# NVlabs/EmerNeRF

Hardware: AMD Instinct MI355X
Metric: train rays/sec (8192-ray batch, 128 samples) (higher is better)
Workload: dtype f32

## Files before the change

### emernerf_amd/_lib.py

```python
from __future__ import annotations

import ctypes
import os
from ctypes import c_float, c_int, c_int32, c_int64, c_uint32, c_uint64, c_void_p

_PKG = os.path.dirname(os.path.abspath(__file__))
LIB_PATH = os.path.join(_PKG, "lib", "libemernerf_hip.so")
EMER_MAX_LEVELS = 32

F32, F16 = 0, 1
ACT_NONE, ACT_RELU, ACT_SIGMOID, ACT_TRUNC_EXP = 0, 1, 2, 3
STOT_TYPES = {"uniform": 0, "uniform_lindisp": 1, "lindisp": 2, "sqrt": 3, "log": 4, "uniform_lindisp_0": 5}


class GridDesc(ctypes.Structure):
    _fields_ = [
        ("n_dims", c_uint32), ("n_levels", c_uint32), ("n_features", c_uint32),
        ("log2_hashmap_size", c_uint32), ("base_resolution", c_uint32), ("per_level_scale", c_float),
        ("scale", c_float * EMER_MAX_LEVELS), ("res", c_uint32 * EMER_MAX_LEVELS),
        ("size", c_uint32 * EMER_MAX_LEVELS), ("offset", c_uint32 * EMER_MAX_LEVELS),
        ("hashed", c_uint32 * EMER_MAX_LEVELS), ("n_entries", c_uint32),
    ]


class EmerError(RuntimeError):
    pass


_P = c_void_p
_GP = ctypes.POINTER(GridDesc)

SIGNATURES = {
    "emer_profile_next": [_P, _P],
    "emer_grid_desc_init": [_GP, c_uint32, c_uint32, c_uint32, c_uint32, c_uint32, c_float],
    "emer_hashgrid_fwd": [_GP, _P, _P, c_int, _P, c_int64, c_int64, _P, c_int64, _P],
    "emer_hashgrid_bwd_params": [_GP, _P, _P, c_int64, c_int64, _P, c_int, c_int64, _P],
    "emer_hashgrid_bwd_params_sliced": [_GP, _P, _P, c_int64, c_int64, _P, _P, c_int64, _P],
    "emer_hashgrid_bwd_params_sliced_add": [_GP, _P, _P, c_int64, c_int64, _P, _P, c_int64, _P],
    "emer_hashgrid_bwd_params_sliced_levels": [_GP, _P, _P, c_int64, c_int64, _P, _P, c_int64, c_int32, c_int32, _P],
    "emer_hashgrid_sliced_split_level": [_GP],
    "emer_hashgrid_sliced_plan": [_GP, _P, _P],
    "emer_hashgrid_slice_masks": [_GP, _P, _P, c_int64, _P],
    "emer_hashgrid_sliced_supported": [_GP],
    "emer_hashgrid_mask_rows": [_P],
    "emer_hashgrid_bwd_input": [_GP, _P, _P, c_int, _P, c_int64, c_int64, _P, c_int64, _P],
    "emer_hashgrid_fwd_jac": [_GP, _P, _P, _P, c_int64, c_int64, _P, _P, c_int64, c_int64, _P],
    "emer_hashgrid_bwd_input_jac": [_GP, _P, _P, c_int64, c_int64, _P, c_int64, _P],
    "emer_layout_transpose": [_P, _P, c_int32, c_int64, c_int32, c_int, _P],
    "emer_contract_fwd": [_P, _P, c_int, _P, c_int64, _P],
    "emer_contract_bwd": [_P, _P, c_int, _P, _P, c_int64, _P],
    "emer_flow_warp_fwd": [_P, _P, _P, _P, _P, c_float, _P, c_int, _P, _P, c_int64, _P],
    "emer_flow_warp_bwd": [_P, _P, _P, _P, c_int, _P, _P, _P, c_int64, _P],
    "emer_ray_points": [_P, _P, _P, _P, _P, _P, c_int, _P, c_int, _P, c_int64, c_int32, _P],
    "emer_importance_sample": [_P, _P, c_int64, c_int32, c_int32, _P, _P, _P, _P, c_float, c_float, c_int, _P],
    "emer_importance_sample_points": [_P, _P, c_int64, c_int32, c_int32, _P, _P, _P, _P, c_float, c_float, c_int, _P, _P, _P, c_int, _P, _P, _P],
    "emer_stot": [_P, c_int64, c_float, c_float, c_int, _P, _P],
    "emer_prop_loss": [_P, _P, c_int32, _P, _P, c_int32, c_float, c_int, c_int64, c_float, _P, _P, c_int, _P, _P],
    "emer_reduce_sum": [_P, c_int64, c_int, _P, _P],
    "emer_scale": [_P, _P, c_float, _P, c_int64, _P],
    "emer_cast_f32_f16": [_P, _P, c_int64, _P],
    "emer_render_weights_fwd": [_P, _P, _P, c_int64, c_int32, _P, _P, _P, _P, _P, _P, _P, _P],
    "emer_render_weights_bwd": [_P, _P, _P, _P, _P, _P, _P, c_int64, c_int32, _P, _P],
    "emer_composite_rgb_fwd": [_P, _P, _P, _P, _P, c_int64, c_int32, _P, _P, _P, _P, _P, _P, _P, _P, _P, _P],
    "emer_composite_rgb_bwd": [_P, _P, _P, _P, _P, _P, _P, _P, _P, _P, _P, _P, c_int64, c_int32, _P, _P, _P, _P],
    "emer_blend_accumulate_fwd": [_P, _P, _P, _P, _P, _P, _P, c_int64, c_int32, _P, _P, _P],
    "emer_blend_accumulate_bwd": [_P, _P, _P, _P, _P, _P, _P, _P, _P, c_int64, c_int32, _P, _P, _P, _P, _P, _P, _P, _P],
    "emer_blend_accumulate_wide_fwd": [_P, _P, _P, _P, _P, _P, c_int64, c_int32, c_int32, _P, _P],
    "emer_blend_accumulate_wide_bwd": [_P, _P, _P, _P, _P, _P, _P, c_int64, c_int32, c_int32, _P, _P, _P, _P, _P, _P, _P],
    "emer_ray_epilogue_fwd": [_P, _P, _P, c_int64, _P, _P, _P, _P, _P],
    "emer_ray_epilogue_bwd": [_P, _P, _P, _P, _P, c_int64, _P, _P, _P],
    "emer_pixel_loss_fwd": [_P, _P, _P, _P, c_int64, c_float, c_float, _P, _P, _P],
    "emer_pixel_loss_bwd": [_P, _P, _P, _P, c_int64, c_float, c_float, _P, _P, _P, _P],
# ... 84 lines not shown
            try:
                fn = getattr(lib, name)
            except AttributeError:
                if ALLOW_MISSING_SYMBOLS:
                    continue
                raise
            fn.argtypes = argtypes
            fn.restype = restype
    lib.emer_last_error.restype = ctypes.c_char_p
    lib.emer_version.restype = c_int
    _lib = lib
    return lib


class KernelTimer:

    def __init__(self, names):
        self.names = set(names)
        self.events = {n: [] for n in self.names}
        self.tags = {n: [] for n in self.names}
        self.ns = {n: [] for n in self.names}
        self.tag = None

    def elapsed_us(self):
        import torch
        torch.cuda.synchronize()
        return {n: [a.elapsed_time(b) * 1e3 for a, b in ev] for n, ev in self.events.items()}


TIMER = None


_N_ARG = {"emer_hashgrid_fwd": 8, "emer_hashgrid_fwd_jac": 9, "emer_hashgrid_bwd_params_sliced": 7, "emer_hashgrid_bwd_params_sliced_add": 7,
          "emer_hashgrid_bwd_params_sliced_levels": 7, "emer_hashgrid_bwd_params": 7, "emer_hashgrid_bwd_input": 8, "emer_hashgrid_bwd_input_jac": 6}
_TIGHT = ("emer_hashgrid_fwd", "emer_hashgrid_fwd_jac", "emer_hashgrid_bwd_params_sliced", "emer_hashgrid_bwd_params_sliced_add", "emer_hashgrid_bwd_params_sliced_levels")


def call(name: str, *args) -> None:
    lib = load()
    t = TIMER
    if t is not None and name in t.names:
        import torch
        a, b = torch.cuda.Event(enable_timing=True), torch.cuda.Event(enable_timing=True)
        a.record()
        if name in _TIGHT:
            b.record()
            lib.emer_profile_next(c_void_p(a.cuda_event), c_void_p(b.cuda_event))
            rc = getattr(lib, name)(*args)
        else:
            rc = getattr(lib, name)(*args)
            b.record()
        t.events[name].append((a, b))
        tag = None
        if name.startswith("emer_hashgrid"):
            d = args[0]._obj
            tag = (d.n_dims, d.n_levels, d.n_features)
        t.tags[name].append(tag)
        t.ns[name].append(int(args[_N_ARG[name]]) if name in _N_ARG else None)
    else:
        rc = getattr(lib, name)(*args)
    if rc != 0:
        raise EmerError(f"{name} failed (rc={rc}): {lib.emer_last_error().decode()}")


def make_grid_desc(n_dims, n_levels, n_features, log2_hashmap_size, base_resolution, per_level_scale) -> GridDesc:
    d = GridDesc()
    call("emer_grid_desc_init", ctypes.byref(d), n_dims, n_levels, n_features, log2_hashmap_size,
         base_resolution, per_level_scale)
# ... 2 lines not shown
```

### emernerf_amd/csrc/hashgrid.hip

```cpp
#include "common.h"

namespace emer {

template <int F, typename PT>
__device__ __forceinline__ void load_feats(const PT *__restrict__ p, float (&v)[F]);

template <> __device__ __forceinline__ void load_feats<1, float>(const float *__restrict__ p, float (&v)[1]) { v[0] = p[0]; }
template <> __device__ __forceinline__ void load_feats<2, float>(const float *__restrict__ p, float (&v)[2]) {
    float2 t = *reinterpret_cast<const float2 *>(p); v[0] = t.x; v[1] = t.y;
}
template <> __device__ __forceinline__ void load_feats<4, float>(const float *__restrict__ p, float (&v)[4]) {
    float4 t = *reinterpret_cast<const float4 *>(p); v[0] = t.x; v[1] = t.y; v[2] = t.z; v[3] = t.w;
}
template <> __device__ __forceinline__ void load_feats<8, float>(const float *__restrict__ p, float (&v)[8]) {
    float4 a = reinterpret_cast<const float4 *>(p)[0], b = reinterpret_cast<const float4 *>(p)[1];
    v[0] = a.x; v[1] = a.y; v[2] = a.z; v[3] = a.w; v[4] = b.x; v[5] = b.y; v[6] = b.z; v[7] = b.w;
}
template <> __device__ __forceinline__ void load_feats<1, __half>(const __half *__restrict__ p, float (&v)[1]) { v[0] = __half2float(p[0]); }
template <> __device__ __forceinline__ void load_feats<2, __half>(const __half *__restrict__ p, float (&v)[2]) {
    float2 t = __half22float2(*reinterpret_cast<const __half2 *>(p)); v[0] = t.x; v[1] = t.y;
}
template <> __device__ __forceinline__ void load_feats<4, __half>(const __half *__restrict__ p, float (&v)[4]) {
    uint2 raw = *reinterpret_cast<const uint2 *>(p);
    float2 a = __half22float2(*reinterpret_cast<__half2 *>(&raw.x)), b = __half22float2(*reinterpret_cast<__half2 *>(&raw.y));
// ... 709 lines not shown
    (void)slice_want; (void)slice_bits;
    const bool on = (uint32_t)lane < count;
    const uint32_t e = on ? Qw[(q_head + (uint32_t)lane) % kPairQueue] : 0u;
    uint32_t n = e >> 8;
    uint32_t match = e & 0xFFu;
    asm volatile("" : "+v"(n));
    float xv[D], go[F], w[D];
    uint32_t gi[D], hd[D][2];
    load_x<D>(x, (int64_t)n, xv);
#pragma unroll
    for (int f = 0; f < F; ++f) go[f] = dl[(int64_t)n * sn + f];
    cell_of<D>(li, xv, gi, w);
    hash_terms<D>(gi, hd);
    add_pair<D, F>(acc, gi, w, hd, go, match, local_mask);
    while (__ballot(match != 0u)) add_pair<D, F>(acc, gi, w, hd, go, match, local_mask);
}

#ifndef EMER_PIPE_K
#define EMER_PIPE_K 2
#endif
template <int D, int F> constexpr int kPipeK() {
    constexpr int per = D + F + 1, k = 28 / per;
    return k > EMER_PIPE_K ? EMER_PIPE_K : (k < 1 ? 1 : k);
}
template <int D, int F, int K>
struct HitGroup {
    float xs[K][D], go[K][F];
    uint32_t ns[K];
    bool vld[K];
    uint32_t take;
};
constexpr int kScanWords = 64 + 64 + 32 + 32;

template <int D, int F>
__global__ __launch_bounds__(kSliceThreads) void hashgrid_bwd_params_sliced_kernel(const emer_grid_desc g, const SlicePlan plan,
                                                                                   const float *__restrict__ x,
                                                                                   const float *__restrict__ dout, int64_t sn, int64_t sl,
                                                                                   const uint64_t *__restrict__ masks,
                                                                                   uint32_t *__restrict__ work_ctr,
                                                                                   float *__restrict__ grad, int64_t N,
                                                                                   uint32_t accumulate) {
    extern __shared__ __attribute__((aligned(16))) double smem[];
    __shared__ uint32_t s_item;
    const uint32_t my_xcd = blockIdx.x & 7u;
    uint8_t *sel_lut = nullptr;
    if constexpr (use_select_lut<D>()) {
    sel_lut = reinterpret_cast<uint8_t *>(reinterpret_cast<uint64_t *>(smem + (size_t)plan.max_local * F) + (size_t)kSliceWaves * kScanWords)
                       + (size_t)kSliceWaves * kPairQueue * sizeof(uint32_t);
    for (uint32_t e = threadIdx.x; e < 2048u; e += kSliceThreads) {
        uint32_t b = e >> 3, k = e & 7u, pos = 0;
        for (uint32_t i = 0; i < 8u; ++i)
            if ((b >> i) & 1u) { if (k == 0u) { pos = i; break; } --k; }
        sel_lut[e] = (uint8_t)pos;
    }
    __syncthreads();
    }
  for (;;) {
    if (threadIdx.x == 0) {
        uint32_t it = 0xFFFFFFFFu;
        for (uint32_t t = 0; t < 8u; ++t) {
            const uint32_t xx = (my_xcd + t) & 7u;
            if (plan.items_per_xcd[xx] == 0u) continue;
            const uint32_t jj = atomicAdd(work_ctr + xx, 1u);
            if (jj < plan.items_per_xcd[xx]) { it = (xx << 24) | jj; break; }
        }
        s_item = it;
    }
    __syncthreads();
    const uint32_t item = s_item;
    __syncthreads();
    if (item == 0xFFFFFFFFu) return;
    const uint32_t xcd = item >> 24;
    uint32_t j = item & 0xFFFFFFu;
    j = ((((j >> plan.sched_shift) << 3) + xcd) << plan.sched_shift) + (j & ((1u << plan.sched_shift) - 1u));
    uint32_t level = 0, slice = 0, range = 0;
    for (uint32_t oi = 0; oi < g.n_levels; ++oi) {
        level = plan.order[oi];
        const uint32_t nb = plan.n_slices[level] * plan.n_ranges[level];
        if (j < nb) { slice = j % plan.n_slices[level]; range = j / plan.n_slices[level]; break; }
        j -= nb;
    }
    const LevelInfo li = level_info(g, level);
#ifdef EMER_SLICED_TRACE
    const unsigned long long trace_t0 = wall_clock64();
    unsigned long long trace_hits = 0;
#endif
    const bool dense_rt = !li.hashed;
    const bool pairable_rt = li.hashed && (li.size & (li.size - 1u)) == 0u && true;
    const bool run_reduced = pairable_rt && F >= 2 && li.res <= (uint32_t)EMER_RUN_RES;
    const bool consecutive = dense_rt || run_reduced || li.res > kStridedHitsMaxRes;
    const uint32_t shift = plan.shift[level], n_ranges = plan.n_ranges[level];
    const uint32_t first = slice << shift;
    const uint32_t n_local = ((li.size - first) < (1u << shift)) ? (li.size - first) : (1u << shift);
    const int64_t n_words = (N + 63) >> 6;
    const int64_t words_per_range = ceil_div_dev(n_words, (int64_t)n_ranges);
    const int64_t w_begin = (int64_t)range * words_per_range;
    const int64_t w_end = (w_begin + words_per_range < n_words) ? w_begin + words_per_range : n_words;

    double *acc = smem;
    const int wave = threadIdx.x >> 6, lane = threadIdx.x & 63;
    uint64_t *scratch = reinterpret_cast<uint64_t *>(smem + (size_t)plan.max_local * F) + (size_t)wave * kScanWords;
    uint64_t *Wl = scratch;
    unsigned long long *Hv = reinterpret_cast<unsigned long long *>(scratch + 64);
    uint32_t *El = reinterpret_cast<uint32_t *>(scratch + 128), *Hx = reinterpret_cast<uint32_t *>(scratch + 160);

    for (uint32_t i = threadIdx.x; i < n_local * F; i += kSliceThreads) acc[i] = 0.0;
    __syncthreads();
    uint32_t *Qw = reinterpret_cast<uint32_t *>(reinterpret_cast<uint64_t *>(smem + (size_t)plan.max_local * F) + (size_t)kSliceWaves * kScanWords)
                   + (size_t)wave * kPairQueue;
    const bool use_queue = pairable_rt && N <= (1ll << kPairQueueShift) && (1u << (D - 1)) <= 8u;
    const uint32_t slice_bits = (li.size - 1u) & ~((1u << shift) - 1u), slice_want = first, local_mask = (1u << shift) - 1u;

    const float *__restrict__ dl = dout + (int64_t)level * sl;
    const uint64_t *__restrict__ bm = masks + ((int64_t)level * (64 * plan.mask_q) + (slice >> plan.gsub[level])) * n_words;
    const uint64_t lt_mask = (1ull << lane) - 1ull;

    auto run_item = [&](auto kind_c) __attribute__((always_inline)) {
    constexpr int KIND = decltype(kind_c)::value;
    constexpr bool dense = KIND == 0, pairable = KIND == 1;
    uint32_t q_head = 0, q_len = 0;
    const int64_t my_word = dense ? (int64_t)lane * kSliceWaves + wave : (int64_t)threadIdx.x;
    const int64_t wave_word0 = dense ? wave : wave * 64;
    const uint32_t lane_word_shift = dense ? (kSliceWaves == 16 ? 4u : 3u) : 0u;
    static_assert(kSliceWaves == 16 || kSliceWaves == 8, "lane_word_shift assumes 16 or 8 waves");
    constexpr int KG = kPipeK<D, F>();
    int64_t wbase = w_begin;
    uint32_t trip_w0 = 0;
    uint32_t total = 0, n_chunks = 0, c0 = 0, hexcl = 0;
    uint64_t hv = 0;
    uint64_t pre = (w_begin + my_word < w_end) ? bm[w_begin + my_word] : 0ull;
    auto next_trip = [&]() __attribute__((always_inline)) -> bool {
        while (wbase < w_end) {
            const uint64_t wv = pre;
            trip_w0 = (uint32_t)wbase;
            wbase += kSliceThreads;
            pre = (wbase + my_word < w_end) ? bm[wbase + my_word] : 0ull;
            const uint32_t p = (uint32_t)__popcll(wv);
            const uint32_t incl = wave_inclusive_sum_u32(p, lane);
            total = (uint32_t)__builtin_amdgcn_readlane((int)incl, 63);
            if (total == 0u) continue;
#ifdef EMER_SLICED_TRACE
            if (lane == 0) trace_hits += total;
// ... 173 lines not shown
            }
        }
        if constexpr (pairable) {
            if (q_len >= kPairQueueDrain) {
                __builtin_amdgcn_fence(__ATOMIC_ACQ_REL, "wavefront");
                const uint32_t done = q_len < 64u ? q_len : 64u;
                drain_pair_queue<D, F>(acc, li, x, dl, sn, Qw, q_head, done, slice_want, slice_bits, local_mask, lane);
                q_head = (q_head + done) % kPairQueue; q_len -= done;
            }
        }
    };
    {
        HitGroup<D, F, KG> ga;
        HitGroup<D, F, KG> gb;
        bool more = issue(ga);
        while (more) {
            const bool more_b = issue(gb);
            consume(ga);
            if (!more_b) break;
            more = issue(ga);
            consume(gb);
        }
    }
    while (q_len) {
        __builtin_amdgcn_fence(__ATOMIC_ACQ_REL, "wavefront");
        const uint32_t done = q_len < 64u ? q_len : 64u;
        drain_pair_queue<D, F>(acc, li, x, dl, sn, Qw, q_head, done, slice_want, slice_bits, local_mask, lane);
        q_head = (q_head + done) % kPairQueue; q_len -= done;
    }
    };
    if (dense_rt) run_item(std::integral_constant<int, 0>{});
    else if (pairable_rt) run_item(std::integral_constant<int, 1>{});
    else run_item(std::integral_constant<int, 2>{});
    __syncthreads();
    float *__restrict__ out = grad + ((size_t)li.offset + first) * F;
    if (n_ranges == 1u) {
        if (accumulate) { for (uint32_t i = threadIdx.x; i < n_local * F; i += kSliceThreads) out[i] += (float)acc[i]; }
        else { for (uint32_t i = threadIdx.x; i < n_local * F; i += kSliceThreads) out[i] = (float)acc[i]; }
    } else {
        for (uint32_t i = threadIdx.x; i < n_local * F; i += kSliceThreads) {
            const float v = (float)acc[i];
            if (v != 0.0f) __hip_atomic_fetch_add(out + i, v, __ATOMIC_RELAXED, __HIP_MEMORY_SCOPE_AGENT);
        }
    }
    __syncthreads();
#ifdef EMER_SLICED_TRACE
    if (g_sliced_trace && threadIdx.x == 0) {
        const unsigned long long slot = atomicAdd(g_sliced_trace, 1ull);
        unsigned long long *rec = g_sliced_trace + 8 + 4 * slot;
        rec[0] = (unsigned long long)level | ((unsigned long long)slice << 8) | ((unsigned long long)range << 24) | ((unsigned long long)blockIdx.x << 40);
        rec[1] = trace_t0; rec[2] = wall_clock64(); rec[3] = trace_hits;
    }
#endif
  }
}

struct ZeroRegions {
    float *p[EMER_MAX_LEVELS + 1];
    uint32_t n[EMER_MAX_LEVELS + 1];
    int32_t count;
};
__global__ __launch_bounds__(256) void zero_regions_kernel(const ZeroRegions z) {
    float *__restrict__ p = z.p[blockIdx.y];
    const uint32_t n = z.n[blockIdx.y];
    for (uint32_t i = blockIdx.x * 256u + threadIdx.x; i < n; i += gridDim.x * 256u) p[i] = 0.0f;
}

template <int D, int Q>
__global__ __launch_bounds__(256) void hashgrid_slice_masks_kernel(const emer_grid_desc g, const SlicePlan plan,
                                                                   const float *__restrict__ x, uint64_t *__restrict__ masks,
                                                                   int64_t N, uint32_t n_chunks, const LevelMap lmap) {
    uint32_t level, chunk;
    if (!map_block(blockIdx.x, lmap, n_chunks, level, chunk)) return;
    const int64_t n = (int64_t)chunk * 256 + threadIdx.x;
    const LevelInfo li = level_info(g, level);
    uint64_t mask[Q];
#pragma unroll
    for (int q = 0; q < Q; ++q) mask[q] = 0ull;
    if (n < N) {
        float xv[D], w[D];
        uint32_t gi[D];
        load_x<D>(x, n, xv);
        cell_of<D>(li, xv, gi, w);
#pragma unroll
        for (uint32_t m = 0; m < (1u << D); ++m) {
            uint32_t c[D];
#pragma unroll
// ... 222 lines not shown
    return make_slice_plan(g).ok ? 1 : 0;
}

extern "C" int emer_hashgrid_mask_rows(const emer_grid_desc *g) {
    if (check_desc(g)) return 0;
    const SlicePlan plan = make_slice_plan(g);
    return plan.ok ? (int)(64u * plan.mask_q) : 0;
}

extern "C" int emer_hashgrid_slice_masks(const emer_grid_desc *g, const float *x, uint64_t *slice_masks, int64_t n, void *stream) {
    if (int rc = check_desc(g)) return rc;
    EMER_REQUIRE(n >= 0, "hashgrid_slice_masks: negative n");
    if (n == 0) return EMER_OK;
    EMER_REQUIRE(x && slice_masks, "hashgrid_slice_masks: null pointer");
    const SlicePlan plan = make_slice_plan(g);
    EMER_REQUIRE(plan.ok, "hashgrid_slice_masks: a level needs more than 256 x 64 LDS slices");
    const uint32_t n_chunks = (uint32_t)ceil_div(n, 256);
    uint32_t blocks = 0;
    const LevelMap lmap = make_level_map(g, n_chunks, &blocks);
    return dispatch_df(g->n_dims, g->n_features, [&](auto d, auto) {
        constexpr int D = decltype(d)::value;
        if (plan.mask_q == 4)
            hipLaunchKernelGGL((hashgrid_slice_masks_kernel<D, 4>), dim3(blocks), dim3(256), 0, as_stream(stream), *g, plan, x, slice_masks, n,
                               n_chunks, lmap);
        else
            hipLaunchKernelGGL((hashgrid_slice_masks_kernel<D, 1>), dim3(blocks), dim3(256), 0, as_stream(stream), *g, plan, x, slice_masks, n,
                               n_chunks, lmap);
        return check_launch("hashgrid_slice_masks");
    });
}

static int hashgrid_bwd_params_sliced_range(const emer_grid_desc *g, const float *x, const float *dout, int64_t sn, int64_t sl,
                                            uint64_t *slice_masks, float *grad, int64_t n, uint32_t level_begin, uint32_t level_end, void *stream,
                                            bool accumulate = false);

extern "C" int emer_hashgrid_bwd_params_sliced(const emer_grid_desc *g, const float *x, const float *dout, int64_t sn,
                                               int64_t sl, uint64_t *slice_masks, float *grad, int64_t n, void *stream) {
    if (int rc = check_desc(g)) return rc;
    return hashgrid_bwd_params_sliced_range(g, x, dout, sn, sl, slice_masks, grad, n, 0u, g->n_levels, stream);
}

extern "C" int emer_hashgrid_bwd_params_sliced_add(const emer_grid_desc *g, const float *x, const float *dout, int64_t sn,
                                                   int64_t sl, uint64_t *slice_masks, float *grad, int64_t n, void *stream) {
    if (int rc = check_desc(g)) return rc;
    return hashgrid_bwd_params_sliced_range(g, x, dout, sn, sl, slice_masks, grad, n, 0u, g->n_levels, stream, true);
}

extern "C" int emer_hashgrid_bwd_params_sliced_levels(const emer_grid_desc *g, const float *x, const float *dout, int64_t sn, int64_t sl,
                                                      uint64_t *slice_masks, float *grad, int64_t n, int32_t level_begin, int32_t level_end,
                                                      void *stream) {
    if (int rc = check_desc(g)) return rc;
    EMER_REQUIRE(level_begin >= 0 && level_begin <= level_end && level_end <= (int32_t)g->n_levels, "hashgrid_bwd_params_sliced_levels: bad level range [%d, %d)",
                 level_begin, level_end);
    if (level_begin == level_end) return EMER_OK;
    return hashgrid_bwd_params_sliced_range(g, x, dout, sn, sl, slice_masks, grad, n, (uint32_t)level_begin, (uint32_t)level_end, stream);
}

extern "C" int emer_hashgrid_sliced_plan(const emer_grid_desc *g, uint32_t *n_slices, uint32_t *n_ranges) {
    if (int rc = check_desc(g)) return rc;
    const SlicePlan plan = make_slice_plan(g);
    EMER_REQUIRE(plan.ok, "hashgrid_sliced_plan: a level needs more than 256 x 64 LDS slices");
    for (uint32_t l = 0; l < g->n_levels; ++l) {
        if (n_slices) n_slices[l] = plan.n_slices[l];
        if (n_ranges) n_ranges[l] = plan.n_ranges[l];
    }
    return (int)plan.total_items;
}

extern "C" int emer_hashgrid_sliced_split_level(const emer_grid_desc *g) {
    if (check_desc(g) != EMER_OK) return 0;
    const SlicePlan plan = make_slice_plan(g);
    if (!plan.ok) return 0;
    const uint32_t owners = 256;
    if (plan.total_items <= owners) return 0;
    uint32_t items = 0, k = g->n_levels;
    while (k > 1u) {
        const uint32_t add = plan.n_slices[k - 1u] * plan.n_ranges[k - 1u];
        if (items + add > owners) break;
        items += add;
        --k;
    }
    return k < g->n_levels ? (int)k : 0;
}

static int hashgrid_bwd_params_sliced_range(const emer_grid_desc *g, const float *x, const float *dout, int64_t sn, int64_t sl,
                                            uint64_t *slice_masks, float *grad, int64_t n, uint32_t level_begin, uint32_t level_end, void *stream,
                                            bool accumulate) {
    EMER_REQUIRE(n >= 0 && n < (1ll << 28), "hashgrid_bwd_params_sliced: n out of range (byte offsets of the gathers are 32-bit: n < 2^28)");
    EMER_REQUIRE(sn == (int64_t)g->n_features, "hashgrid_bwd_params_sliced: dout must be level-major with packed features (stride_n == n_features)");
    EMER_REQUIRE(x && dout && grad && slice_masks, "hashgrid_bwd_params_sliced: null pointer");
    const uint32_t F = g->n_features;
    SlicePlan plan = make_slice_plan(g);
    EMER_REQUIRE(plan.ok, "hashgrid_bwd_params_sliced: a level needs more than 256 x 64 LDS slices; use emer_hashgrid_bwd_params");
    if (level_begin != 0u || level_end != g->n_levels) {
        uint32_t left_items = 0;
        for (uint32_t l = 0; l < g->n_levels; ++l) {
            if (l < level_begin || l >= level_end) plan.n_slices[l] = 0;
            left_items += plan.n_slices[l] * plan.n_ranges[l];
        }
        plan.total_items = left_items;
        for (int i = 0; i < 8; ++i) plan.items_per_xcd[i] = 0;
        const uint32_t sched_block = 1u << plan.sched_shift;
        for (uint32_t blk = 0; blk * sched_block < left_items; ++blk) {
            const uint32_t left = left_items - blk * sched_block;
            plan.items_per_xcd[blk & 7u] += left < sched_block ? left : sched_block;
        }
    }
    uint32_t total_items = 0;
    for (int i = 0; i < 8; ++i) total_items += plan.items_per_xcd[i];
    if (total_items == 0u) return EMER_OK;
    ZeroRegions zr;
    zr.count = 0;
    uint32_t *work_ctr = reinterpret_cast<uint32_t *>(slice_masks + (size_t)g->n_levels * (64 * plan.mask_q) * (size_t)ceil_div(n, 64));
    zr.p[zr.count] = reinterpret_cast<float *>(work_ctr); zr.n[zr.count] = 8u; ++zr.count;
    for (uint32_t l = level_begin; l < level_end; ++l) {
        if (plan.n_ranges[l] > 1u && !accumulate) {
            zr.p[zr.count] = grad + (size_t)g->offset[l] * F; zr.n[zr.count] = g->size[l] * F; ++zr.count;
        }
    }
    hipLaunchKernelGGL(zero_regions_kernel, dim3(64, (uint32_t)zr.count), dim3(256), 0, as_stream(stream), zr);
    if (int rc = check_launch("hashgrid_bwd_params_sliced(zero)")) return rc;
    uint32_t n_blocks = 256;
    if (total_items < n_blocks) n_blocks = (total_items + 7u) / 8u * 8u;
    const size_t lds_base = (size_t)plan.max_local * F * sizeof(double) + (size_t)kSliceWaves * (kScanWords * sizeof(uint64_t) + kPairQueue * sizeof(uint32_t));
    return dispatch_df(g->n_dims, g->n_features, [&](auto d, auto f) {
        constexpr int D = decltype(d)::value, FF = decltype(f)::value;
        auto kern = hashgrid_bwd_params_sliced_kernel<D, FF>;
        const size_t lds = lds_base + select_lut_bytes<D>();
        if (int rc = reserve_lds(reinterpret_cast<const void *>(kern), lds, "hashgrid_bwd_params_sliced")) return rc;
        const ProfileEvents ev = take_profile_events();
        EMER_LAUNCH_PROFILED(ev, kern, dim3(n_blocks), dim3(kSliceThreads), lds, as_stream(stream), *g, plan, x, dout, sn, sl,
                           slice_masks, work_ctr, grad, n, accumulate ? 1u : 0u);
        return check_launch("hashgrid_bwd_params_sliced");
    });
}

#ifdef EMER_SLICED_TRACE
extern "C" int emer_debug_sliced_trace(unsigned long long *buf) {
    return hipMemcpyToSymbol(HIP_SYMBOL(g_sliced_trace), &buf, sizeof(buf)) == hipSuccess ? EMER_OK : EMER_E_LAUNCH;
}
#endif

extern "C" int emer_hashgrid_bwd_input(const emer_grid_desc *g, const float *x, const void *params, int param_dtype,
                                       const float *dout, int64_t sn, int64_t sl, float *dx, int64_t n, void *stream) {
    if (int rc = check_desc(g)) return rc;
    EMER_REQUIRE(n >= 0, "hashgrid_bwd_input: negative n");
    if (n == 0) return EMER_OK;
    EMER_REQUIRE(x && params && dout && dx, "hashgrid_bwd_input: null pointer");
    EMER_REQUIRE(param_dtype == EMER_F32 || param_dtype == EMER_F16, "hashgrid_bwd_input: bad param_dtype %d", param_dtype);
    const uint32_t blocks = (uint32_t)ceil_div(n, 256);
    return dispatch_df(g->n_dims, g->n_features, [&](auto d, auto f) {
        constexpr int D = decltype(d)::value, F = decltype(f)::value;
        if (param_dtype == EMER_F32)
            hipLaunchKernelGGL((hashgrid_bwd_input_kernel<D, F, float>), dim3(blocks), dim3(256), 0, as_stream(stream), *g, x,
                               (const float *)params, dout, sn, sl, dx, n);
        else
            hipLaunchKernelGGL((hashgrid_bwd_input_kernel<D, F, __half>), dim3(blocks), dim3(256), 0, as_stream(stream), *g,
                               x, (const __half *)params, dout, sn, sl, dx, n);
        return check_launch("hashgrid_bwd_input");
    });
}
```

### emernerf_amd/ops.py

```python
from __future__ import annotations

import ctypes
import os
from typing import Optional, Tuple

import torch
from torch import Tensor

from . import _lib
from ._lib import ACT_NONE, ACT_RELU, ACT_SIGMOID, ACT_TRUNC_EXP, F16, F32, GridDesc, STOT_TYPES

_ACTS = {None: ACT_NONE, "none": ACT_NONE, "relu": ACT_RELU, "sigmoid": ACT_SIGMOID, "trunc_exp": ACT_TRUNC_EXP}


def _ptr(t: Optional[Tensor]):
    return None if t is None else ctypes.c_void_p(t.data_ptr())


def _stream(t: Tensor):
    return ctypes.c_void_p(torch.cuda.current_stream(t.device).cuda_stream)


def _check_cuda(*ts: Tensor):
    for t in ts:
        if t is not None and not t.is_cuda:
            raise _lib.EmerError("emernerf_amd ops need GPU (HIP) tensors; there is no CPU fallback")


def _ng(*args):
    if torch.is_grad_enabled():
        return args
    return tuple(a.detach() if isinstance(a, Tensor) else a for a in args)


# ... 163 lines not shown
                              _ptr(grad), N, st)
                else:
                    grad = torch.zeros(pc.numel(), device=xc.device, dtype=gdt)
                    _lib.call("emer_hashgrid_bwd_params", ctypes.byref(desc), _ptr(xc), _ptr(dlm), F, N * F, _ptr(grad),
                              _dtype_tag(grad), N, st)
                dp = _table_grad_via_autograd(ctx.param_obj, grad.to(pc.dtype) if grad.dtype != pc.dtype else grad)
            if ctx.needs_input_grad[0]:
                dx = torch.empty_like(xc)
                _lib.call("emer_hashgrid_bwd_input", ctypes.byref(desc), _ptr(xc), _ptr(pc), _dtype_tag(pc), _ptr(dlm), F,
                          N * F, _ptr(dx), N, st)
        return dx, dp, None, None


def _count_table_eval(param) -> None:
    if getattr(param, "_emer_before_table_grad", None) is not None or getattr(param, "_emer_after_table_grad", None) is not None:
        param._emer_pending_evals = getattr(param, "_emer_pending_evals", 0) + 1


def _before_table_grad(param) -> bool:
    cb, after = getattr(param, "_emer_before_table_grad", None), getattr(param, "_emer_after_table_grad", None)
    if cb is None and after is None:
        return False
    left = getattr(param, "_emer_pending_evals", 1) - 1
    param._emer_pending_evals = max(left, 0)
    if left <= 0 and cb is not None:
        cb()
    return left <= 0


def _after_table_grad(param, last: bool, in_place: bool) -> None:
    cb = getattr(param, "_emer_after_table_grad", None)
    if cb is not None and last and in_place:
        cb(param)


class _HashGridLMFn(torch.autograd.Function):

    @staticmethod
    def forward(ctx, x: Tensor, params: Tensor, desc: GridDesc, grad_dtype, table_dtype=None, skip_dx_rows: int = 0):
        xc, pc = _f32c(x), params.detach().contiguous()
        if table_dtype == torch.float16 and pc.dtype == torch.float32:
            ph = torch.empty(pc.shape, device=pc.device, dtype=torch.float16)
            with torch.cuda.device(pc.device):
                _lib.call("emer_cast_f32_f16", _ptr(pc), _ptr(ph), pc.numel(), _stream(pc))
            pc = ph
        gdt = grad_dtype or torch.float32
        ctx.sliced = bool(ctx.needs_input_grad[1] and gdt == torch.float32 and sliced_supported(desc))
        k = min(int(skip_dx_rows), xc.shape[0])
        jac = None
        if GRID_JAC and ctx.needs_input_grad[0] and pc.dtype == torch.float32 and k < xc.shape[0] and _jac_fits(desc, xc.shape[0] - k):
            res = hashgrid_fwd_raw(desc, xc, pc, level_major=True, want_masks=ctx.sliced, jac_row0=k)
            lm, masks, jac = res if ctx.sliced else (res[0], None, res[1])
        elif ctx.sliced:
            lm, masks = hashgrid_fwd_raw(desc, xc, pc, level_major=True, want_masks=True)
        else:
            lm, masks = hashgrid_fwd_raw(desc, xc, pc, level_major=True), None
        ctx.jac = jac
        ctx.desc, ctx.grad_dtype = desc, grad_dtype
        ctx.skip_dx_rows = int(skip_dx_rows)
        ctx.master_dtype = params.dtype
        from . import fused
        sink = fused._sink(params) if ctx.sliced else None
        ctx.param = params if (sink is not None and sink.is_contiguous() and sink.numel() == pc.numel()) else None
        ctx.param_obj = params
        _count_table_eval(params)
        ctx.save_for_backward(xc, pc, masks)
        return lm

    @staticmethod
    def backward(ctx, dlm: Tensor):
        xc, pc, masks = ctx.saved_tensors
        desc = ctx.desc
        N, L, F = xc.shape[0], desc.n_levels, desc.n_features
        dx = dp = None
        last = _before_table_grad(ctx.param_obj)
        with torch.cuda.device(xc.device):
            dlm = _f32c(dlm)
            if CHECK_FINITE:
                _check_finite_grid_grad(dlm, desc)
            st = _stream(xc)
            if ctx.needs_input_grad[1]:
                gdt = ctx.grad_dtype or torch.float32
                if gdt == torch.float32 and masks is not None:
                    param = ctx.param
                    direct = param is not None and getattr(param, "_emer_grad_fresh", False) and param.grad is not None
                    add = (not direct) and param is not None and param.grad is not None and param.grad.is_contiguous()
                    grad = param.grad.view(-1) if (direct or add) else torch.empty(pc.numel(), device=xc.device, dtype=torch.float32)
                    split = getattr(ctx.param_obj, "_emer_table_split", None) if (direct and last) else None
                    if split is not None and 0 < split[0] < L:
                        k, hook = split
                        _lib.call("emer_hashgrid_bwd_params_sliced_levels", ctypes.byref(desc), _ptr(xc), _ptr(dlm), F, N * F, _ptr(masks),
                                  _ptr(grad), N, k, L, st)
                        hook(param, int(desc.offset[k]) * F, pc.numel())
                        _lib.call("emer_hashgrid_bwd_params_sliced_levels", ctypes.byref(desc), _ptr(xc), _ptr(dlm), F, N * F, _ptr(masks),
                                  _ptr(grad), N, 0, k, st)
                    else:
                        _lib.call("emer_hashgrid_bwd_params_sliced_add" if add else "emer_hashgrid_bwd_params_sliced", ctypes.byref(desc), _ptr(xc),
                                  _ptr(dlm), F, N * F, _ptr(masks), _ptr(grad), N, st)
                    if direct:
                        param._emer_grad_fresh = False
                        grad = None
                    elif add:
                        grad = None
                    elif param is not None and param.grad is not None:
                        param.grad.view(-1).add_(grad)
                        grad = None
                else:
                    grad = torch.zeros(pc.numel(), device=xc.device, dtype=gdt)
                    _lib.call("emer_hashgrid_bwd_params", ctypes.byref(desc), _ptr(xc), _ptr(dlm), F, N * F, _ptr(grad),
                              _dtype_tag(grad), N, st)
                dp = None if grad is None else _table_grad_via_autograd(ctx.param_obj, grad.to(ctx.master_dtype) if grad.dtype != ctx.master_dtype else grad)
                _after_table_grad(ctx.param_obj, last, dp is None)
            if ctx.needs_input_grad[0]:
                k, D = min(ctx.skip_dx_rows, N), desc.n_dims
                dx = torch.empty_like(xc)
                if k > 0:
                    dx[:k].zero_()
                if N > k and ctx.jac is not None:
                    _lib.call("emer_hashgrid_bwd_input_jac", ctypes.byref(desc), _ptr(ctx.jac), dlm.data_ptr() + 4 * k * F, F, N * F,
                              dx.data_ptr() + 4 * k * D, N - k, st)
                    ctx.jac = None
                elif N > k:
                    _lib.call("emer_hashgrid_bwd_input", ctypes.byref(desc), xc.data_ptr() + 4 * k * D, _ptr(pc), _dtype_tag(pc),
                              dlm.data_ptr() + 4 * k * F, F, N * F, dx.data_ptr() + 4 * k * D, N - k, st)
        return dx, dp, None, None, None, None


def hashgrid_encode_lm(x: Tensor, params: Tensor, desc: GridDesc, grad_dtype=None, table_dtype=None, skip_dx_rows: int = 0) -> Tensor:
    return _HashGridLMFn.apply(*_ng(x, params, desc, grad_dtype, table_dtype, skip_dx_rows))


def hashgrid_encode(x: Tensor, params: Tensor, desc: GridDesc, grad_dtype=None) -> Tensor:
# ... 789 lines not shown
```

### emernerf_amd/prop_net.py

```python
from __future__ import annotations

import logging
from typing import Callable, List, Optional, Sequence, Tuple

import torch
from torch import Tensor

from . import ops
from .nerfacc_compat import AbstractEstimator, RayIntervals

logger = logging.getLogger()


class PropNetEstimator(AbstractEstimator):

    def __init__(self, optimizer: Optional[torch.optim.Optimizer] = None, scheduler=None,
                 enable_anti_aliasing_loss: Optional[bool] = True,
                 anti_aliasing_pulse_width: Optional[List[float]] = [0.03, 0.003]) -> None:
        super().__init__()
        self.optimizer, self.scheduler = optimizer, scheduler
        self.prop_cache: List = []
        self.enable_anti_aliasing_loss = enable_anti_aliasing_loss
        self.pulse_width = anti_aliasing_pulse_width
        self.jitter_fn: Optional[Callable[[int, torch.device], Tensor]] = None
# ... 1 lines not shown

    @torch.no_grad()
    def sampling(self, prop_sigma_fns: List[Callable], prop_samples: List[int], num_samples: int, n_rays: int,
                 near_plane: float, far_plane: float, sampling_type: str = "uniform_lindisp",
                 stratified: bool = False, requires_grad: bool = False, ray_geometry=None) -> Tuple[Tensor, Tensor]:
        assert len(prop_sigma_fns) == len(prop_samples), \
            "The number of proposal networks and the number of samples should be the same."
        dev = self.device
        planes = (float(near_plane), float(far_plane), sampling_type)
        key = (int(n_rays), str(dev))
        unit = self._unit.get(key)
        if unit is None:
            if torch.cuda.is_available() and dev.type == "cuda" and torch.cuda.is_current_stream_capturing():
                unit = torch.arange(2, device=dev, dtype=torch.float32).expand(n_rays, 2).contiguous()
            else:
                unit = self._unit[key] = torch.arange(2, device=dev, dtype=torch.float32).expand(n_rays, 2).contiguous()
        edges = cdfs = unit
        jitters = None
        if stratified and self.jitter_fn is None:
            jitters = iter(torch.rand((len(prop_samples) + 1, n_rays), device=dev).unbind(0))
        draw = (lambda: next(jitters)) if jitters is not None else (lambda: self.jitter_fn(n_rays, dev))
        def sample(edges_in, cdfs_in, n_out, u, slot):
            geo = None
            if ray_geometry is not None and ops.SAMPLE_POINTS and 2 * edges_in.shape[-1] + n_out + 1 <= ops.sample_points_capacity():
                geo = ray_geometry[2][slot]
            if geo is None:
                return ops.importance_sample(edges_in, cdfs_in, n_out, u, stot=planes, intervals=True)
            aabb, unbounded, want_pos = geo
            e, a, b, normed, pos = ops.importance_sample(edges_in, cdfs_in, n_out, u, stot=planes, intervals=True,
                                                         points=(ray_geometry[0], ray_geometry[1], aabb, unbounded, want_pos))
            a._emer_points = (normed, pos, aabb, bool(unbounded))
            return e, a, b

        for level, (sigma_fn, n_level) in enumerate(zip(prop_sigma_fns, prop_samples)):
            u = draw() if stratified else None
            edges, t0, t1 = sample(edges, cdfs, n_level, u, level)
            with torch.set_grad_enabled(requires_grad):
                sigma = sigma_fn(t0, t1)["density"].squeeze(-1)
                assert sigma.shape == t0.shape
                cdfs = ops.render_weights(t0, t1, sigma)[3]
            if requires_grad:
                self.prop_cache.append((RayIntervals(vals=edges), cdfs, level))
            else:
                cdfs = cdfs.detach()
        u = draw() if stratified else None
        edges, t0, t1 = sample(edges, cdfs.detach(), num_samples, u, len(prop_samples))
        if requires_grad:
            self.prop_cache.append((RayIntervals(vals=edges), None, None))
        return t0, t1

    @torch.enable_grad()
    def compute_loss(self, trans: Tensor, loss_scaler: float = 1.0) -> Tensor:
        if not self.prop_cache:
            return torch.zeros((), device=self.device)
        final, _, _ = self.prop_cache.pop()
        s_final = final.vals
        R, n = trans.shape
        anti = bool(self.enable_anti_aliasing_loss)
        trans_ng = trans.detach()
        total = None
        while self.prop_cache:
            level_edges, level_cdfs, level = self.prop_cache.pop()
            m = level_cdfs.shape[-1] - 1
            count = R * (m if anti else n)
            pulse = float(self.pulse_width[level]) if anti else 0.0
            term = ops.prop_level_loss(s_final, trans_ng, level_edges.vals, level_cdfs, pulse, anti, float(loss_scaler) / count)
            total = term if total is None else total + term
        return total if total is not None else torch.zeros((), device=self.device)

    @torch.enable_grad()
    def update_every_n_steps(self, trans: Tensor, requires_grad: bool = False, loss_scaler: float = 1.0) -> float:
        if not requires_grad:
            if self.scheduler is not None:
                self.scheduler.step()
            return 0.0
        return self._update(trans=trans, loss_scaler=loss_scaler)

# ... 38 lines not shown
```

### include/emernerf_hip.h

```cpp
#ifndef EMERNERF_HIP_H
#define EMERNERF_HIP_H

#include <stdint.h>

#ifdef __cplusplus
extern "C" {
#endif

#define EMER_MAX_LEVELS 32

#define EMER_OK 0
#define EMER_E_INVALID (-1)
#define EMER_E_LAUNCH (-2)

#define EMER_F32 0
#define EMER_F16 1

#define EMER_ACT_NONE 0
#define EMER_ACT_RELU 1
#define EMER_ACT_SIGMOID 2
#define EMER_ACT_TRUNC_EXP 3

#define EMER_STOT_UNIFORM 0
#define EMER_STOT_UNIFORM_LINDISP 1
// ... 14 lines not shown
    uint32_t base_resolution;
    float per_level_scale;
    float scale[EMER_MAX_LEVELS];
    uint32_t res[EMER_MAX_LEVELS];
    uint32_t size[EMER_MAX_LEVELS];
    uint32_t offset[EMER_MAX_LEVELS];
    uint32_t hashed[EMER_MAX_LEVELS];
    uint32_t n_entries;
} emer_grid_desc;

int emer_grid_desc_init(emer_grid_desc *host_desc, uint32_t n_dims, uint32_t n_levels,
                        uint32_t n_features, uint32_t log2_hashmap_size, uint32_t base_resolution,
                        float per_level_scale);

#define EMER_SLICE_MASK_SCRATCH 2064
int emer_hashgrid_fwd(const emer_grid_desc *host_desc, const float *x, const void *params,
                      int param_dtype, float *out, int64_t out_stride_n, int64_t out_stride_l,
                      uint64_t *slice_masks, int64_t n, void *stream);

int emer_hashgrid_bwd_params(const emer_grid_desc *host_desc, const float *x, const float *dout,
                             int64_t dout_stride_n, int64_t dout_stride_l, void *grad,
                             int grad_dtype, int64_t n, void *stream);

int emer_hashgrid_bwd_params_sliced(const emer_grid_desc *host_desc, const float *x,
                                    const float *dout, int64_t dout_stride_n,
                                    int64_t dout_stride_l, uint64_t *slice_masks,
                                    float *grad, int64_t n, void *stream);
int emer_hashgrid_sliced_plan(const emer_grid_desc *g, uint32_t *n_slices, uint32_t *n_ranges);
int emer_hashgrid_bwd_params_sliced_add(const emer_grid_desc *g, const float *x, const float *dout, int64_t stride_n,
                                        int64_t stride_l, uint64_t *slice_masks, float *grad, int64_t n, void *stream);
int emer_hashgrid_bwd_params_sliced_levels(const emer_grid_desc *host_desc, const float *x, const float *dout,
                                           int64_t dout_stride_n, int64_t dout_stride_l, uint64_t *slice_masks,
                                           float *grad, int64_t n, int32_t level_begin, int32_t level_end, void *stream);
int emer_hashgrid_sliced_split_level(const emer_grid_desc *host_desc);
int emer_hashgrid_slice_masks(const emer_grid_desc *host_desc, const float *x,
                              uint64_t *slice_masks, int64_t n, void *stream);
int emer_hashgrid_sliced_supported(const emer_grid_desc *host_desc);
int emer_hashgrid_mask_rows(const emer_grid_desc *host_desc);

int emer_hashgrid_bwd_input(const emer_grid_desc *host_desc, const float *x, const void *params,
                            int param_dtype, const float *dout, int64_t dout_stride_n,
                            int64_t dout_stride_l, float *dx, int64_t n, void *stream);
int emer_hashgrid_fwd_jac(const emer_grid_desc *host_desc, const float *x, const float *params, float *out,
                          int64_t out_stride_n, int64_t out_stride_l, uint64_t *slice_masks, float *jac,
                          int64_t jac_row0, int64_t n, void *stream);
int emer_hashgrid_bwd_input_jac(const emer_grid_desc *host_desc, const float *jac, const float *dout,
                                int64_t dout_stride_n, int64_t dout_stride_l, float *dx, int64_t n_rows, void *stream);

int emer_layout_transpose(const float *src, float *dst, int32_t n_levels, int64_t n,
                          int32_t n_features, int to_row_major, void *stream);

int emer_contract_fwd(const float *pos, const float *aabb, int unbounded, float *out, int64_t n,
                      void *stream);
int emer_contract_bwd(const float *pos, const float *aabb, int unbounded, const float *dout,
                      float *dpos, int64_t n, void *stream);
int emer_flow_warp_fwd(const float *positions, const float *normed, const float *timestamps, const float *flow,
                       const float *noise, float time_diff, const float *aabb, int unbounded, float *x3, float *x2,
                       int64_t n, void *stream);
int emer_flow_warp_bwd(const float *positions, const float *flow, const float *noise, const float *aabb, int unbounded,
                       const float *dx3, const float *dx2, float *dflow, int64_t n, void *stream);
int emer_ray_points(const float *origins, const float *dirs, const float *t_starts,
                    const float *t_ends, const float *times, const float *aabb, int unbounded,
                    float *normed, int out_dim, float *positions_out, int64_t n_rays,
                    int32_t n_samples, void *stream);

int64_t emer_importance_sample_points_capacity(void);
// ... 283 lines not shown
```

Measured before the change: 3.489 million.

## Pair proposal-level hash table backward passes into one two-segment sliced kernel

When the same hash-grid table is evaluated several times inside the proposal sampling loop, the first backward call stashes its inputs and the next one launches a two-segment sliced kernel. That kernel accumulates both point sets into the same LDS slice before a single write-out. This halves the number of sliced gradient scatters, and with them the LDS zeroing and flush passes over the table, for the proposal networks. In exchange it adds cross-call state in autograd, a queued flush callback for leftover stashes, and more code complexity in the kernel.

```diff
diff --git a/emernerf_amd/_lib.py b/emernerf_amd/_lib.py
--- a/emernerf_amd/_lib.py
+++ b/emernerf_amd/_lib.py
@@ -38,6 +38,7 @@
     "emer_hashgrid_bwd_params_sliced": [_GP, _P, _P, c_int64, c_int64, _P, _P, c_int64, _P],
     "emer_hashgrid_bwd_params_sliced_add": [_GP, _P, _P, c_int64, c_int64, _P, _P, c_int64, _P],
     "emer_hashgrid_bwd_params_sliced_levels": [_GP, _P, _P, c_int64, c_int64, _P, _P, c_int64, c_int32, c_int32, _P],
+    "emer_hashgrid_bwd_params_sliced2": [_GP, _P, _P, _P, c_int64, _P, _P, _P, c_int64, c_int64, _P, c_int32, c_int32, c_int32, _P],
     "emer_hashgrid_sliced_split_level": [_GP],
     "emer_hashgrid_sliced_plan": [_GP, _P, _P],
     "emer_hashgrid_slice_masks": [_GP, _P, _P, c_int64, _P],
@@ -188,8 +189,9 @@
 
 
 _N_ARG = {"emer_hashgrid_fwd": 8, "emer_hashgrid_fwd_jac": 9, "emer_hashgrid_bwd_params_sliced": 7, "emer_hashgrid_bwd_params_sliced_add": 7,
-          "emer_hashgrid_bwd_params_sliced_levels": 7, "emer_hashgrid_bwd_params": 7, "emer_hashgrid_bwd_input": 8, "emer_hashgrid_bwd_input_jac": 6}
-_TIGHT = ("emer_hashgrid_fwd", "emer_hashgrid_fwd_jac", "emer_hashgrid_bwd_params_sliced", "emer_hashgrid_bwd_params_sliced_add", "emer_hashgrid_bwd_params_sliced_levels")
+          "emer_hashgrid_bwd_params_sliced_levels": 7, "emer_hashgrid_bwd_params_sliced2": 4, "emer_hashgrid_bwd_params": 7, "emer_hashgrid_bwd_input": 8, "emer_hashgrid_bwd_input_jac": 6}
+_TIGHT = ("emer_hashgrid_fwd", "emer_hashgrid_fwd_jac", "emer_hashgrid_bwd_params_sliced", "emer_hashgrid_bwd_params_sliced_add", "emer_hashgrid_bwd_params_sliced_levels",
+          "emer_hashgrid_bwd_params_sliced2")
 
 
 def call(name: str, *args) -> None:
diff --git a/emernerf_amd/csrc/hashgrid.hip b/emernerf_amd/csrc/hashgrid.hip
--- a/emernerf_amd/csrc/hashgrid.hip
+++ b/emernerf_amd/csrc/hashgrid.hip
@@ -765,14 +765,19 @@
 };
 constexpr int kScanWords = 64 + 64 + 32 + 32;
 
-template <int D, int F>
-__global__ __launch_bounds__(kSliceThreads) void hashgrid_bwd_params_sliced_kernel(const emer_grid_desc g, const SlicePlan plan,
-                                                                                   const float *__restrict__ x,
-                                                                                   const float *__restrict__ dout, int64_t sn, int64_t sl,
-                                                                                   const uint64_t *__restrict__ masks,
-                                                                                   uint32_t *__restrict__ work_ctr,
-                                                                                   float *__restrict__ grad, int64_t N,
-                                                                                   uint32_t accumulate) {
+struct SlicedSeg {
+    const float *x;
+    const float *dout;
+    int64_t sl;
+    const uint64_t *masks;
+    int64_t n;
+};
+
+template <int D, int F, int NSEG>
+__device__ __forceinline__ void hashgrid_bwd_params_sliced_body(const emer_grid_desc &g, const SlicePlan &plan, const float *__restrict__ x,
+                                                                const float *__restrict__ dout, int64_t sn, int64_t sl,
+                                                                const uint64_t *__restrict__ masks, uint32_t *__restrict__ work_ctr,
+                                                                float *__restrict__ grad, int64_t N, uint32_t accumulate, const SlicedSeg &seg1) {
     extern __shared__ __attribute__((aligned(16))) double smem[];
     __shared__ uint32_t s_item;
     const uint32_t my_xcd = blockIdx.x & 7u;
@@ -825,10 +830,6 @@
     const uint32_t shift = plan.shift[level], n_ranges = plan.n_ranges[level];
     const uint32_t first = slice << shift;
     const uint32_t n_local = ((li.size - first) < (1u << shift)) ? (li.size - first) : (1u << shift);
-    const int64_t n_words = (N + 63) >> 6;
-    const int64_t words_per_range = ceil_div_dev(n_words, (int64_t)n_ranges);
-    const int64_t w_begin = (int64_t)range * words_per_range;
-    const int64_t w_end = (w_begin + words_per_range < n_words) ? w_begin + words_per_range : n_words;
 
     double *acc = smem;
     const int wave = threadIdx.x >> 6, lane = threadIdx.x & 63;
@@ -841,6 +842,12 @@
     __syncthreads();
     uint32_t *Qw = reinterpret_cast<uint32_t *>(reinterpret_cast<uint64_t *>(smem + (size_t)plan.max_local * F) + (size_t)kSliceWaves * kScanWords)
                    + (size_t)wave * kPairQueue;
+    auto run_seg = [&](const float *__restrict__ x, const float *__restrict__ dout, int64_t sl, const uint64_t *__restrict__ masks,
+                       int64_t N) __attribute__((always_inline)) {
+    const int64_t n_words = (N + 63) >> 6;
+    const int64_t words_per_range = ceil_div_dev(n_words, (int64_t)n_ranges);
+    const int64_t w_begin = (int64_t)range * words_per_range;
+    const int64_t w_end = (w_begin + words_per_range < n_words) ? w_begin + words_per_range : n_words;
     const bool use_queue = pairable_rt && N <= (1ll << kPairQueueShift) && (1u << (D - 1)) <= 8u;
     const uint32_t slice_bits = (li.size - 1u) & ~((1u << shift) - 1u), slice_want = first, local_mask = (1u << shift) - 1u;
 
@@ -1080,6 +1087,9 @@
     if (dense_rt) run_item(std::integral_constant<int, 0>{});
     else if (pairable_rt) run_item(std::integral_constant<int, 1>{});
     else run_item(std::integral_constant<int, 2>{});
+    };
+    run_seg(x, dout, sl, masks, N);
+    if constexpr (NSEG == 2) run_seg(seg1.x, seg1.dout, seg1.sl, seg1.masks, seg1.n);
     __syncthreads();
     float *__restrict__ out = grad + ((size_t)li.offset + first) * F;
     if (n_ranges == 1u) {
@@ -1101,6 +1111,29 @@
     }
 #endif
   }
+}
+
+template <int D, int F>
+__global__ __launch_bounds__(kSliceThreads) void hashgrid_bwd_params_sliced_kernel(const emer_grid_desc g, const SlicePlan plan,
+                                                                                   const float *__restrict__ x,
+                                                                                   const float *__restrict__ dout, int64_t sn, int64_t sl,
+                                                                                   const uint64_t *__restrict__ masks,
+                                                                                   uint32_t *__restrict__ work_ctr,
+                                                                                   float *__restrict__ grad, int64_t N,
+                                                                                   uint32_t accumulate) {
+    const SlicedSeg none{nullptr, nullptr, 0, nullptr, 0};
+    hashgrid_bwd_params_sliced_body<D, F, 1>(g, plan, x, dout, sn, sl, masks, work_ctr, grad, N, accumulate, none);
+}
+
+template <int D, int F>
+__global__ __launch_bounds__(kSliceThreads) void hashgrid_bwd_params_sliced2_kernel(const emer_grid_desc g, const SlicePlan plan,
+                                                                                    const float *__restrict__ x,
+                                                                                    const float *__restrict__ dout, int64_t sn, int64_t sl,
+                                                                                    const uint64_t *__restrict__ masks,
+                                                                                    uint32_t *__restrict__ work_ctr,
+                                                                                    float *__restrict__ grad, int64_t N,
+                                                                                    uint32_t accumulate, const SlicedSeg seg1) {
+    hashgrid_bwd_params_sliced_body<D, F, 2>(g, plan, x, dout, sn, sl, masks, work_ctr, grad, N, accumulate, seg1);
 }
 
 struct ZeroRegions {
@@ -1389,7 +1422,7 @@
 
 static int hashgrid_bwd_params_sliced_range(const emer_grid_desc *g, const float *x, const float *dout, int64_t sn, int64_t sl,
                                             uint64_t *slice_masks, float *grad, int64_t n, uint32_t level_begin, uint32_t level_end, void *stream,
-                                            bool accumulate = false);
+                                            bool accumulate = false, const SlicedSeg *seg1 = nullptr);
 
 extern "C" int emer_hashgrid_bwd_params_sliced(const emer_grid_desc *g, const float *x, const float *dout, int64_t sn,
                                                int64_t sl, uint64_t *slice_masks, float *grad, int64_t n, void *stream) {
@@ -1411,6 +1444,20 @@
                  level_begin, level_end);
     if (level_begin == level_end) return EMER_OK;
     return hashgrid_bwd_params_sliced_range(g, x, dout, sn, sl, slice_masks, grad, n, (uint32_t)level_begin, (uint32_t)level_end, stream);
+}
+
+extern "C" int emer_hashgrid_bwd_params_sliced2(const emer_grid_desc *g, const float *x0, const float *dout0, uint64_t *masks0, int64_t n0,
+                                                const float *x1, const float *dout1, const uint64_t *masks1, int64_t n1, int64_t sn,
+                                                float *grad, int32_t level_begin, int32_t level_end, int32_t accumulate, void *stream) {
+    if (int rc = check_desc(g)) return rc;
+    EMER_REQUIRE(level_begin >= 0 && level_begin <= level_end && level_end <= (int32_t)g->n_levels, "hashgrid_bwd_params_sliced2: bad level range [%d, %d)",
+                 level_begin, level_end);
+    EMER_REQUIRE(n1 >= 0 && n1 < (1ll << 28), "hashgrid_bwd_params_sliced2: n1 out of range (byte offsets of the gathers are 32-bit: n < 2^28)");
+    EMER_REQUIRE(x1 && dout1 && masks1, "hashgrid_bwd_params_sliced2: null pointer");
+    if (level_begin == level_end) return EMER_OK;
+    const SlicedSeg seg1{x1, dout1, n1 * sn, masks1, n1};
+    return hashgrid_bwd_params_sliced_range(g, x0, dout0, sn, n0 * sn, masks0, grad, n0, (uint32_t)level_begin, (uint32_t)level_end, stream,
+                                            accumulate != 0, &seg1);
 }
 
 extern "C" int emer_hashgrid_sliced_plan(const emer_grid_desc *g, uint32_t *n_slices, uint32_t *n_ranges) {
@@ -1442,7 +1489,7 @@
 
 static int hashgrid_bwd_params_sliced_range(const emer_grid_desc *g, const float *x, const float *dout, int64_t sn, int64_t sl,
                                             uint64_t *slice_masks, float *grad, int64_t n, uint32_t level_begin, uint32_t level_end, void *stream,
-                                            bool accumulate) {
+                                            bool accumulate, const SlicedSeg *seg1) {
     EMER_REQUIRE(n >= 0 && n < (1ll << 28), "hashgrid_bwd_params_sliced: n out of range (byte offsets of the gathers are 32-bit: n < 2^28)");
     EMER_REQUIRE(sn == (int64_t)g->n_features, "hashgrid_bwd_params_sliced: dout must be level-major with packed features (stride_n == n_features)");
     EMER_REQUIRE(x && dout && grad && slice_masks, "hashgrid_bwd_params_sliced: null pointer");
@@ -1482,10 +1529,17 @@
     const size_t lds_base = (size_t)plan.max_local * F * sizeof(double) + (size_t)kSliceWaves * (kScanWords * sizeof(uint64_t) + kPairQueue * sizeof(uint32_t));
     return dispatch_df(g->n_dims, g->n_features, [&](auto d, auto f) {
         constexpr int D = decltype(d)::value, FF = decltype(f)::value;
+        const size_t lds = lds_base + select_lut_bytes<D>();
+        const ProfileEvents ev = take_profile_events();
+        if (seg1) {
+            auto kern = hashgrid_bwd_params_sliced2_kernel<D, FF>;
+            if (int rc = reserve_lds(reinterpret_cast<const void *>(kern), lds, "hashgrid_bwd_params_sliced2")) return rc;
+            EMER_LAUNCH_PROFILED(ev, kern, dim3(n_blocks), dim3(kSliceThreads), lds, as_stream(stream), *g, plan, x, dout, sn, sl,
+                                 slice_masks, work_ctr, grad, n, accumulate ? 1u : 0u, *seg1);
+            return check_launch("hashgrid_bwd_params_sliced2");
+        }
         auto kern = hashgrid_bwd_params_sliced_kernel<D, FF>;
-        const size_t lds = lds_base + select_lut_bytes<D>();
         if (int rc = reserve_lds(reinterpret_cast<const void *>(kern), lds, "hashgrid_bwd_params_sliced")) return rc;
-        const ProfileEvents ev = take_profile_events();
         EMER_LAUNCH_PROFILED(ev, kern, dim3(n_blocks), dim3(kSliceThreads), lds, as_stream(stream), *g, plan, x, dout, sn, sl,
                            slice_masks, work_ctr, grad, n, accumulate ? 1u : 0u);
         return check_launch("hashgrid_bwd_params_sliced");
diff --git a/emernerf_amd/ops.py b/emernerf_amd/ops.py
--- a/emernerf_amd/ops.py
+++ b/emernerf_amd/ops.py
@@ -1,5 +1,6 @@
 from __future__ import annotations
 
+import contextlib
 import ctypes
 import os
 from typing import Optional, Tuple
@@ -229,6 +230,53 @@
     cb = getattr(param, "_emer_after_table_grad", None)
     if cb is not None and last and in_place:
         cb(param)
+
+
+PAIR_TABLE_BWD = os.environ.get("EMER_PAIR_TABLE_BWD", "1") != "0"
+_PAIR_SCOPE: Optional[dict] = None
+
+
+class _TableBwdPair:
+    __slots__ = ("pending", "stash")
+
+    def __init__(self):
+        self.pending, self.stash = 0, None
+
+
+@contextlib.contextmanager
+def paired_table_backward(enabled: bool = True):
+    global _PAIR_SCOPE
+    prev = _PAIR_SCOPE
+    _PAIR_SCOPE = {} if (enabled and PAIR_TABLE_BWD) else None
+    try:
+        yield
+    finally:
+        _PAIR_SCOPE = prev
+
+
+def _sliced_bwd(desc, xc, dlm, masks, grad, seg1, lo: int, hi: int, add: bool, st) -> None:
+    N, L, F = xc.shape[0], desc.n_levels, desc.n_features
+    if seg1 is not None:
+        x1, d1, m1 = seg1
+        _lib.call("emer_hashgrid_bwd_params_sliced2", ctypes.byref(desc), _ptr(xc), _ptr(dlm), _ptr(masks), N, _ptr(x1), _ptr(d1), _ptr(m1),
+                  x1.shape[0], F, _ptr(grad), lo, hi, int(add), st)
+    elif (lo, hi) != (0, L):
+        _lib.call("emer_hashgrid_bwd_params_sliced_levels", ctypes.byref(desc), _ptr(xc), _ptr(dlm), F, N * F, _ptr(masks), _ptr(grad), N, lo, hi, st)
+    else:
+        _lib.call("emer_hashgrid_bwd_params_sliced_add" if add else "emer_hashgrid_bwd_params_sliced", ctypes.byref(desc), _ptr(xc), _ptr(dlm),
+                  F, N * F, _ptr(masks), _ptr(grad), N, st)
+
+
+def _flush_pair(pair: _TableBwdPair, desc, param) -> None:
+    if pair.stash is None:
+        return
+    xc, dlm, masks = pair.stash
+    pair.stash = None
+    direct = getattr(param, "_emer_grad_fresh", False)
+    with torch.cuda.device(xc.device):
+        _sliced_bwd(desc, xc, dlm, masks, param.grad.view(-1), None, 0, desc.n_levels, not direct, _stream(xc))
+    if direct:
+        param._emer_grad_fresh = False
 
 
 class _HashGridLMFn(torch.autograd.Function):
@@ -260,6 +308,10 @@
         sink = fused._sink(params) if ctx.sliced else None
         ctx.param = params if (sink is not None and sink.is_contiguous() and sink.numel() == pc.numel()) else None
         ctx.param_obj = params
+        ctx.pair = None
+        if ctx.param is not None and _PAIR_SCOPE is not None:
+            ctx.pair = _PAIR_SCOPE.setdefault(id(params), _TableBwdPair())
+            ctx.pair.pending += 1
         _count_table_eval(params)
         ctx.save_for_backward(xc, pc, masks)
         return lm
@@ -282,19 +334,30 @@
                     param = ctx.param
                     direct = param is not None and getattr(param, "_emer_grad_fresh", False) and param.grad is not None
                     add = (not direct) and param is not None and param.grad is not None and param.grad.is_contiguous()
-                    grad = param.grad.view(-1) if (direct or add) else torch.empty(pc.numel(), device=xc.device, dtype=torch.float32)
+                    pair, seg1, stashed = ctx.pair, None, False
+                    if pair is not None:
+                        pair.pending -= 1
+                        if pair.stash is not None:
+                            seg1, pair.stash = pair.stash, None
+                        elif pair.pending > 0 and not last and (direct or add):
+                            pair.stash, stashed = (xc, dlm, masks), True
+                            pdesc = desc
+                            torch.autograd.Variable._execution_engine.queue_callback(lambda: _flush_pair(pair, pdesc, param))
+                    grad = None if stashed else param.grad.view(-1) if (direct or add) else \
+                        torch.empty(pc.numel(), device=xc.device, dtype=torch.float32)
                     split = getattr(ctx.param_obj, "_emer_table_split", None) if (direct and last) else None
-                    if split is not None and 0 < split[0] < L:
+                    if stashed:
+                        pass
+                    elif split is not None and 0 < split[0] < L:
                         k, hook = split
-                        _lib.call("emer_hashgrid_bwd_params_sliced_levels", ctypes.byref(desc), _ptr(xc), _ptr(dlm), F, N * F, _ptr(masks),
-                                  _ptr(grad), N, k, L, st)
+                        _sliced_bwd(desc, xc, dlm, masks, grad, seg1, k, L, False, st)
                         hook(param, int(desc.offset[k]) * F, pc.numel())
-                        _lib.call("emer_hashgrid_bwd_params_sliced_levels", ctypes.byref(desc), _ptr(xc), _ptr(dlm), F, N * F, _ptr(masks),
-                                  _ptr(grad), N, 0, k, st)
+                        _sliced_bwd(desc, xc, dlm, masks, grad, seg1, 0, k, False, st)
                     else:
-                        _lib.call("emer_hashgrid_bwd_params_sliced_add" if add else "emer_hashgrid_bwd_params_sliced", ctypes.byref(desc), _ptr(xc),
-                                  _ptr(dlm), F, N * F, _ptr(masks), _ptr(grad), N, st)
-                    if direct:
+                        _sliced_bwd(desc, xc, dlm, masks, grad, seg1, 0, L, add, st)
+                    if stashed:
+                        pass
+                    elif direct:
                         param._emer_grad_fresh = False
                         grad = None
                     elif add:
diff --git a/emernerf_amd/prop_net.py b/emernerf_amd/prop_net.py
--- a/emernerf_amd/prop_net.py
+++ b/emernerf_amd/prop_net.py
@@ -57,17 +57,18 @@
             a._emer_points = (normed, pos, aabb, bool(unbounded))
             return e, a, b
 
-        for level, (sigma_fn, n_level) in enumerate(zip(prop_sigma_fns, prop_samples)):
-            u = draw() if stratified else None
-            edges, t0, t1 = sample(edges, cdfs, n_level, u, level)
-            with torch.set_grad_enabled(requires_grad):
-                sigma = sigma_fn(t0, t1)["density"].squeeze(-1)
-                assert sigma.shape == t0.shape
-                cdfs = ops.render_weights(t0, t1, sigma)[3]
-            if requires_grad:
-                self.prop_cache.append((RayIntervals(vals=edges), cdfs, level))
-            else:
-                cdfs = cdfs.detach()
+        with ops.paired_table_backward(requires_grad):
+            for level, (sigma_fn, n_level) in enumerate(zip(prop_sigma_fns, prop_samples)):
+                u = draw() if stratified else None
+                edges, t0, t1 = sample(edges, cdfs, n_level, u, level)
+                with torch.set_grad_enabled(requires_grad):
+                    sigma = sigma_fn(t0, t1)["density"].squeeze(-1)
+                    assert sigma.shape == t0.shape
+                    cdfs = ops.render_weights(t0, t1, sigma)[3]
+                if requires_grad:
+                    self.prop_cache.append((RayIntervals(vals=edges), cdfs, level))
+                else:
+                    cdfs = cdfs.detach()
         u = draw() if stratified else None
         edges, t0, t1 = sample(edges, cdfs.detach(), num_samples, u, len(prop_samples))
         if requires_grad:
diff --git a/include/emernerf_hip.h b/include/emernerf_hip.h
--- a/include/emernerf_hip.h
+++ b/include/emernerf_hip.h
@@ -70,6 +70,9 @@
 int emer_hashgrid_bwd_params_sliced_levels(const emer_grid_desc *host_desc, const float *x, const float *dout,
                                            int64_t dout_stride_n, int64_t dout_stride_l, uint64_t *slice_masks,
                                            float *grad, int64_t n, int32_t level_begin, int32_t level_end, void *stream);
+int emer_hashgrid_bwd_params_sliced2(const emer_grid_desc *host_desc, const float *x0, const float *dout0, uint64_t *masks0, int64_t n0,
+                                     const float *x1, const float *dout1, const uint64_t *masks1, int64_t n1, int64_t dout_stride_n,
+                                     float *grad, int32_t level_begin, int32_t level_end, int32_t accumulate, void *stream);
 int emer_hashgrid_sliced_split_level(const emer_grid_desc *host_desc);
 int emer_hashgrid_slice_masks(const emer_grid_desc *host_desc, const float *x,
                               uint64_t *slice_masks, int64_t n, void *stream);
```

Measured after the change: 3.489 million (median of 4 runs). No clear change (-0.0%).
